# tonychang04/distributed-machine-learning-cluster

Hardware: AMD Instinct MI355X
Metric: images/sec (whole node) + p50/p95 query latency, ResNet18 ImageNet (higher is better)
Workload: dtype bf16

## Files before the change

### csrc/bindings/py_module.cpp

```cpp
#include <pybind11/numpy.h>
#include <pybind11/pybind11.h>
#include "../serve/shard.h"
#include <pybind11/stl.h>

#include <map>

#include "../kernels/kernels.h"
#include "../runtime/engine.h"
#include "../runtime/jpeg.h"
#include "../runtime/jpeg_gpu.h"
#include "../runtime/ot_io.h"

namespace py = pybind11;
using namespace dmlc;

namespace {

template <typename T>
T* P(uintptr_t v) {
  return reinterpret_cast<T*>(v);
}
hipStream_t S(uintptr_t v) { return reinterpret_cast<hipStream_t>(v); }

WeightMap to_weight_map(const py::dict& d) {
// ... 216 lines not shown
    maxpool2d(P<void>(x), P<void>(y), B, H, W, C, conv_out_dim(H, k, stride, pad),
              conv_out_dim(W, k, stride, pad), k, stride, pad, S(stream));
  });
  m.def("avgpool_global", [](uintptr_t x, uintptr_t y, int B, int HW, int C, uintptr_t stream) {
    avgpool_global(P<void>(x), P<void>(y), B, HW, C, S(stream));
  });
  m.def("avgpool_adaptive", [](uintptr_t x, uintptr_t y, int B, int H, int W, int C, int Ho, int Wo,
                               uintptr_t stream) {
    avgpool_adaptive(P<void>(x), P<void>(y), B, H, W, C, Ho, Wo, S(stream));
  });
  m.def(
      "preprocess_u8",
      [](uintptr_t x, uintptr_t y, int B, int Hin, int Win, int S_, int pad, int Wr, uintptr_t stream,
         bool paired) { preprocess_u8(P<uint8_t>(x), P<void>(y), B, Hin, Win, S_, pad, Wr, S(stream), paired); },
      py::arg("x"), py::arg("y"), py::arg("B"), py::arg("Hin"), py::arg("Win"), py::arg("S"), py::arg("pad"),
      py::arg("Wr"), py::arg("stream"), py::arg("paired") = false);
  m.attr("STEM_POOL_K") = kStemPoolK;
  m.def("stem_pool_pick_strip", &stem_pool_pick_strip);
  m.def("stem_pool_u8_pick_strip", &stem_pool_u8_pick_strip);
  m.def("conv3x3_stream_supported", &conv3x3_stream_supported, py::arg("Hin"), py::arg("Win"), py::arg("Cin"),
        py::arg("Cout"), py::arg("stride") = 1);
  m.def("conv3x3_stream", [](uintptr_t x, uintptr_t w, uintptr_t bias, uintptr_t res, uintptr_t y, uintptr_t zero,
                             int B, int H, int W, int Cin, int Cout, int stride, bool relu, uintptr_t stream,
                             uintptr_t stamps, uintptr_t wd, uintptr_t bd, uintptr_t yd, uintptr_t wfrag,
                             uintptr_t wdfrag) {
    conv3x3_stream(P<void>(x), P<void>(w), P<float>(bias), P<void>(res), P<void>(y), P<void>(zero), B, H, W, Cin, Cout,
                   stride, relu, S(stream), P<unsigned long long>(stamps), P<void>(wd), P<float>(bd), P<void>(yd),
                   P<void>(wfrag), P<void>(wdfrag));
  }, py::arg("x"), py::arg("w"), py::arg("bias"), py::arg("res"), py::arg("y"), py::arg("zero"), py::arg("B"),
        py::arg("H"), py::arg("W"), py::arg("Cin"), py::arg("Cout"), py::arg("stride"), py::arg("relu"),
        py::arg("stream"), py::arg("stamps") = 0, py::arg("wd") = 0, py::arg("bd") = 0, py::arg("yd") = 0,
        py::arg("wfrag") = 0, py::arg("wdfrag") = 0);
  m.def("conv3x3_stream_uses_frag", &conv3x3_stream_uses_frag);
  m.def("conv3x3_stream_set_variant", &conv3x3_stream_set_variant);
  m.def("conv3x3_rows_supported", &conv3x3_rows_supported);
  m.def("conv3x3_rows_pick_strip", &conv3x3_rows_pick_strip);
  m.def("conv3x3_rows", [](uintptr_t x, uintptr_t w, uintptr_t bias, uintptr_t res, uintptr_t y, uintptr_t zero,
                           int B, int H, int W, int C, bool relu, int strip, uintptr_t stream, uintptr_t wfrag) {
    conv3x3_rows(P<void>(x), P<void>(w), P<float>(bias), P<void>(res), P<void>(y), P<void>(zero), B, H, W, C, relu,
                 strip, S(stream), P<void>(wfrag));
  }, py::arg("x"), py::arg("w"), py::arg("bias"), py::arg("res"), py::arg("y"), py::arg("zero"), py::arg("B"),
        py::arg("H"), py::arg("W"), py::arg("C"), py::arg("relu"), py::arg("strip"), py::arg("stream"),
        py::arg("wfrag") = 0);
  m.def("conv3x3_block_supported", &conv3x3_block_supported);
  m.def("conv3x3_block", [](uintptr_t x, uintptr_t wf1, uintptr_t b1, uintptr_t wf2, uintptr_t b2, uintptr_t y,
                            uintptr_t zero, int B, uintptr_t stream) {
    conv3x3_block(P<void>(x), P<void>(wf1), P<float>(b1), P<void>(wf2), P<float>(b2), P<void>(y), P<void>(zero), B,
                  S(stream));
  }, py::arg("x"), py::arg("wf1"), py::arg("b1"), py::arg("wf2"), py::arg("b2"), py::arg("y"), py::arg("zero"),
        py::arg("B"), py::arg("stream"));
  m.def("bottleneck56", [](uintptr_t x, uintptr_t w1, uintptr_t a1, uintptr_t b1, uintptr_t wf2, uintptr_t b2,
                           uintptr_t wf3, uintptr_t b3, uintptr_t y, float res_scale, float out_inv_scale, int B,
                           uintptr_t stream) {
    bottleneck56(P<void>(x), P<void>(w1), P<float>(a1), P<float>(b1), P<void>(wf2), P<float>(b2), P<void>(wf3),
                 P<float>(b3), P<void>(y), res_scale, out_inv_scale, B, S(stream));
  }, py::arg("x"), py::arg("w1"), py::arg("a1"), py::arg("b1"), py::arg("wf2"), py::arg("b2"), py::arg("wf3"),
     py::arg("b3"), py::arg("y"), py::arg("res_scale"), py::arg("out_inv_scale"), py::arg("B"), py::arg("stream") = 0);
  m.def("conv3x3_stream8_supported", &conv3x3_stream8_supported);
  m.def("conv3x3_stream8_frag_offset", &conv3x3_stream8_frag_offset);
  m.def("conv3x3_stream8_set_variant", &conv3x3_stream8_set_variant);
  m.def("conv3x3_stream8", [](uintptr_t x, uintptr_t wf, uintptr_t alpha, uintptr_t bias, uintptr_t y, uintptr_t zero,
                              int B, int H, int W, int Cin, int Cout, int stride, bool relu, float out_inv_scale,
                              uintptr_t stream) {
    conv3x3_stream8(P<void>(x), P<void>(wf), P<float>(alpha), P<float>(bias), P<void>(y), P<void>(zero), B, H, W, Cin,
                    Cout, stride, relu, out_inv_scale, S(stream));
  }, py::arg("x"), py::arg("wf"), py::arg("alpha"), py::arg("bias"), py::arg("y"), py::arg("zero"), py::arg("B"),
// ... 244 lines not shown
          "from_ot",
          [](const std::string& arch, const std::string& path, int device, int num_classes, int image_size,
             const std::map<std::string, bool>& options) {
            return new Engine(arch, ot_load(path), device, num_classes, image_size, engine_options(options));
          },
          py::arg("arch"), py::arg("path"), py::arg("device") = 0, py::arg("num_classes") = 1000,
          py::arg("image_size") = 224, py::arg("options") = std::map<std::string, bool>{})
      .def("reserve", &Engine::reserve, py::call_guard<py::gil_scoped_release>())
      .def(
          "forward",
          [](Engine& e, uintptr_t images, int B, int Hin, int Win, uintptr_t idx, uintptr_t prob,
             uintptr_t logits, uintptr_t stream, bool use_graph) {
            e.forward(P<uint8_t>(images), B, Hin, Win, P<int32_t>(idx), P<float>(prob), P<float>(logits),
                      S(stream), use_graph);
          },
          py::arg("images"), py::arg("B"), py::arg("Hin"), py::arg("Win"), py::arg("idx"),
          py::arg("prob"), py::arg("logits"), py::arg("stream"), py::arg("use_graph") = true,
          py::call_guard<py::gil_scoped_release>())
      .def(
          "forward_topk",
          [](Engine& e, uintptr_t images, int B, int Hin, int Win, int k, uintptr_t idx, uintptr_t prob,
             uintptr_t logits, uintptr_t stream, bool use_graph) {
            e.forward_topk(P<uint8_t>(images), B, Hin, Win, k, P<int32_t>(idx), P<float>(prob), P<float>(logits),
                           S(stream), use_graph);
          },
          py::arg("images"), py::arg("B"), py::arg("Hin"), py::arg("Win"), py::arg("k"), py::arg("idx"),
          py::arg("prob"), py::arg("logits"), py::arg("stream"), py::arg("use_graph") = true,
          py::call_guard<py::gil_scoped_release>())
      .def("profile",
           [](Engine& e, uintptr_t images, int B, int Hin, int Win, uintptr_t stream) {
             return e.profile(P<uint8_t>(images), B, Hin, Win, S(stream));
           })
      .def("activation_ptr", [](const Engine& e, int id) { return reinterpret_cast<uintptr_t>(e.activation(id)); })
      .def("activation_shape",
           [](const Engine& e, int id) {
             auto s = e.activation_shape(id);
             return py::make_tuple(s.H, s.W, s.C, s.f32);
           })
      .def("op_list", [=](const Engine& e) { return op_list(e.ops()); })
      .def("plan", [=](const Engine& e, int B, int Hin, int Win, int topk) {
        return plan_list(e.plan_lines(e.plan(B, Hin, Win, topk)));
      }, py::arg("B"), py::arg("Hin"), py::arg("Win"), py::arg("topk") = 1)
      .def_property_readonly("num_cus", &Engine::num_cus)
      .def_property_readonly("num_activations", &Engine::num_activations)
      .def_property_readonly("arch", &Engine::arch)
      .def_property_readonly("device", &Engine::device)
      .def_property_readonly("num_classes", &Engine::num_classes)
      .def_property_readonly("image_size", &Engine::image_size)
      .def_property_readonly("max_batch", &Engine::max_batch)
      .def_property_readonly("weight_bytes", &Engine::weight_bytes)
      .def_property_readonly("activation_bytes", &Engine::activation_bytes)
      .def_property_readonly("gflop_per_image", &Engine::gflop_per_image);

  bind_dp(m);
}
```

### csrc/kernels/conv3x3_stream.hip

```cpp
#include <atomic>

#include "common.h"
#include "kernels.h"

namespace dmlc {

namespace {

template <int N>
__device__ __forceinline__ void vm_wait() {
  static_assert(N >= 0 && N < 64, "vmcnt range");
  asm volatile("s_waitcnt vmcnt(%0)" ::"i"(N) : "memory");
}

struct StreamConvArgs {
  const bf16* x;
  const bf16* w;
  const float* bias;
  const bf16* res;
  bf16* y;
  const bf16* zero;
  const bf16* wd;
  const float* bd;
  bf16* yd;
// ... 425 lines not shown
}

template <int H, int W, int CI, int CO, int HS, int IMG, int NSP, int WM, int S, bool WR = false, int PD = 4,
          int NG = 1, int PRIO = 0>
void launch_stream(const StreamConvArgs& a, hipStream_t s) {
  using G = StreamGeom<H, W, CI, HS, IMG, S, 3>;
  constexpr size_t lds = WR ? (size_t)G::XBYTES : G::LDS;
  static_assert(lds <= 160 * 1024, "LDS budget");
  const int grid = (a.B + IMG - 1) / IMG * (H / HS) * NSP;
  if constexpr (WR) {
    if constexpr (S == 2) {
      if (a.yd) {
        hipLaunchKernelGGL((conv3x3_stream_kernel<H, W, CI, CO, HS, IMG, NSP, WM, S, 3, true, true, PD, NG, PRIO>),
                           dim3(grid), dim3(512), lds, s, a);
        return;
      }
    }
      hipLaunchKernelGGL((conv3x3_stream_kernel<H, W, CI, CO, HS, IMG, NSP, WM, S, 3, false, true, PD, NG, PRIO>),
                         dim3(grid), dim3(512), lds, s, a);
    return;
  } else {
    if constexpr (S == 2) {
      if (a.yd) {
        hipLaunchKernelGGL((conv3x3_stream_kernel<H, W, CI, CO, HS, IMG, NSP, WM, S, 3, true, false>), dim3(grid),
                           dim3(512), lds, s, a);
        return;
      }
    }
    hipLaunchKernelGGL((conv3x3_stream_kernel<H, W, CI, CO, HS, IMG, NSP, WM, S, 3, false, false>), dim3(grid),
                       dim3(512), lds, s, a);
  }
}

std::atomic<int> g_stream_variant{0};

}

void conv3x3_stream_set_variant(int v) { g_stream_variant = v; }

bool conv3x3_stream_pool_supported(int Hin, int Win, int Cin, int Cout, int stride) {
  return stride == 1 && Hin == 7 && Win == 7 && Cin == 512 && Cout == 512;
}

bool conv3x3_stream_supported(int Hin, int Win, int Cin, int Cout, int stride) {
  if (stride == 1)
    return Cin == Cout && ((Hin == 28 && Win == 28 && Cin == 128) || (Hin == 14 && Win == 14 && Cin == 256) ||
                           (Hin == 7 && Win == 7 && Cin == 512) || (Hin == 56 && Win == 56 && Cin == 64));
  if (stride == 2)
    return (Cout == 2 * Cin && ((Hin == 56 && Win == 56 && Cin == 64) || (Hin == 28 && Win == 28 && Cin == 128) ||
                                (Hin == 14 && Win == 14 && Cin == 256))) ||
           (Cout == Cin && Hin == 56 && Win == 56 && Cin == 128);
  return false;
}

bool conv3x3_stream_uses_frag(int Hin, int Win, int Cin, int Cout, int stride) {
  if (stride == 2)
    return (Cout == 2 * Cin && ((Hin == 28 && Win == 28 && Cin == 128) || (Hin == 14 && Cin == 256))) ||
           (Cout == Cin && Hin == 56 && Win == 56 && Cin == 128);
  return stride == 1 && Cin == Cout && ((Hin == 7 && Win == 7 && Cin == 512) || (Hin == 14 && Win == 14 && Cin == 256));
}

void conv3x3_stream(const void* x, const void* w, const float* bias, const void* res, void* y, const void* zero,
                    int B, int Hin, int Win, int Cin, int Cout, int stride, bool relu, hipStream_t s,
                    unsigned long long* stamps, const void* wd, const float* bd, void* yd, const void* wfrag,
                    const void* wdfrag, void* pool, bool store_y, float out_inv_scale) {
  if (B <= 0) return;
  if (out_inv_scale > 0.f && (res || pool || yd || !store_y))
    throw std::invalid_argument("conv3x3_stream: e4m3 output without residual, pool or downsample only");
  if ((pool || !store_y) && !conv3x3_stream_pool_supported(Hin, Win, Cin, Cout, stride))
    throw std::invalid_argument("conv3x3_stream: fused avgpool needs whole-image workgroups");
  if (pool && ((uintptr_t)pool & 15)) throw std::invalid_argument("conv3x3_stream: misaligned pool");
  if (!conv3x3_stream_supported(Hin, Win, Cin, Cout, stride))
    throw std::invalid_argument("conv3x3_stream: unsupported shape");
  if (!x || !w || !bias || !y || !zero ||
      (((uintptr_t)x | (uintptr_t)w | (uintptr_t)y | (uintptr_t)zero | (uintptr_t)res) & 15))
    throw std::invalid_argument("conv3x3_stream: null / misaligned operand");
  StreamConvArgs a;
  a.x = (const bf16*)x;
  a.w = (const bf16*)w;
  a.bias = bias;
  a.res = (const bf16*)res;
  a.y = (bf16*)y;
  a.zero = (const bf16*)zero;
  a.B = B;
  a.relu = relu;
  a.stamps = stamps;
  a.stagger = kernel_stagger(kStagStream);
  a.wd = (const bf16*)wd;
  a.bd = bd;
  a.yd = (bf16*)yd;
  a.wf = (const bf16*)wfrag;
  a.wdf = (const bf16*)wdfrag;
// ... 52 lines not shown
```

### csrc/kernels/kernels.h

```cpp
#pragma once
#include <hip/hip_runtime.h>
#include <stdint.h>
#include <stdexcept>
#include <string>

namespace dmlc {

#define DMLC_HIP_CHECK(expr)                                                          \
  do {                                                                                \
    hipError_t _e = (expr);                                                           \
    if (_e != hipSuccess)                                                             \
      throw std::runtime_error(std::string("HIP error ") + hipGetErrorString(_e) +    \
                               " at " + __FILE__ + ":" + std::to_string(__LINE__)); \
  } while (0)

struct ConvArgs {
  const void* x = nullptr;
  const void* w = nullptr;
  const void* zero = nullptr;
  const float* bias = nullptr;
  const void* res = nullptr;
  void* y = nullptr;
  int B = 0, H = 0, W = 0, Cin = 0;
  int Ho = 0, Wo = 0, KH = 1, KW = 1, stride = 1, pad = 0;
// ... 100 lines not shown
void bottleneck56_head(const void* x, const void* w1, const float* b1, const void* wf2, const float* b2, void* y,
                       int B, hipStream_t s);
bool conv3x3_s2rows_supported(int Hin, int Win, int Cin, int Cout);
bool conv3x3_s2rows128_supported(int Hin, int Win, int Cin, int Cout);
void conv3x3_s2rows128(const void* x, const void* wf, const float* bias, void* y, int B, bool relu,
                       float out_inv_scale, hipStream_t s);
void conv3x3_s2rows(const void* x, const void* wf, const float* bias, const void* wdf, const float* bd, void* y,
                    void* yd, const void* zero, int B, bool relu, hipStream_t s);
bool conv3x3_rows28_supported(int H, int W, int Cin, int Cout);
void conv3x3_rows28(const void* x, const void* wf, const float* bias, const void* res, void* y, int B, bool relu,
                    hipStream_t s, float out_inv_scale = 0.f, const void* xds = nullptr,
                    const void* wds = nullptr, const float* bds = nullptr);
bool conv_small_supported(int H, int W, int CI, int CO, int stride);
int conv_small_pick_mf(int B, int H, int W, int CI, int CO, int stride, int num_cus);
void conv_small_set_mf(int mf);
void conv_small(const void* x, const void* wf, const float* bias, const void* res, void* y, int B, int H, int W,
                int CI, int CO, int stride, bool relu, int mf, hipStream_t s, const void* wdf = nullptr,
                const float* bd = nullptr, void* yd = nullptr);
bool conv3x3_stream_supported(int Hin, int Win, int Cin, int Cout, int stride = 1);
bool conv3x3_stream8_supported(int Hin, int Win, int Cin, int Cout, int stride = 1);
size_t conv3x3_stream8_frag_offset(int j, int t, int nf, int h, int lane, int KT);
void conv3x3_stream8(const void* x, const void* wf, const float* alpha, const float* bias, void* y, const void* zero,
                     int B, int Hin, int Win, int Cin, int Cout, int stride, bool relu, float out_inv_scale,
                     hipStream_t s);
void conv3x3_stream8_set_variant(int v);
void conv3x3_stream(const void* x, const void* w, const float* bias, const void* res, void* y, const void* zero,
                    int B, int Hin, int Win, int Cin, int Cout, int stride, bool relu, hipStream_t s,
                    unsigned long long* stamps = nullptr, const void* wd = nullptr, const float* bd = nullptr,
                    void* yd = nullptr, const void* wfrag = nullptr, const void* wdfrag = nullptr,
                    void* pool = nullptr, bool store_y = true, float out_inv_scale = 0.f);
bool conv3x3_stream_pool_supported(int Hin, int Win, int Cin, int Cout, int stride);
bool conv3x3_stream_uses_frag(int Hin, int Win, int Cin, int Cout, int stride);
void conv3x3_stream_set_variant(int v);
inline size_t stream_frag_index(int n, int k, int K) {
  const int g = n / 32, r = n % 32;
  const int nf = (r >> 2) & 1, rr = ((r >> 3) << 2) | (r & 3);
  const int t = k / 32, kk = k % 32, lane = (kk / 8) * 16 + rr, e = kk % 8;
  return ((((size_t)g * (K / 32) + t) * 2 + nf) * 64 + lane) * 8 + e;
}
int stem_pool_pick_strip(int B, int PH, int num_cus);
int stem_pool_u8_pick_strip(int B, int PH, int num_cus);
void stem_conv_pool(const void* x, const void* w, const float* bias, void* y, int B, int S, int Wq, int strip,
                    hipStream_t s);
void stem_conv_pool_set_dbg(int dbg);
void stem_conv_pool_set_stamps(void* p);
enum StaggerKernel { kStagStream = 0, kStagBlock, kStagRows28, kStagS2rows, kStagStem, kStagStream8, kStagConv1x1,
                     kStagBottleneck, kStagCount };
int kernel_stagger(int k);
void kernel_stagger_set(int k, int n);
void kernel_stagger_for_lanes(int lanes);
void stem_conv_pool_u8(const uint8_t* x, const void* w, const float* bias, void* y, int B, int S, int strip,
                       hipStream_t s, const void* w_dense = nullptr);
constexpr int kStemDenseK = 160;
struct StemDenseCell {
  int dy, u;
  bool pad;
};
constexpr StemDenseCell stem_dense_cell(int j, int fq) {
  if (j < 15) return {2 * (j / 5) + (fq & 1), 2 * (j % 5) + (fq >> 1), false};
  const int hp = 2 * (j - 15) + (fq >> 1), m = fq & 1;
  if (hp < 3) return {2 * hp + m, 10, false};
  if (hp < 6) return {m ? 5 : 6, hp - 3, m == 1};
  return {6, 3 + 2 * (hp - 6) + m, false};
}
inline int stem_dense_k_index(int dy, int dx, int c) {
  const int e = 3 * dx + c, u = e / 2, h = e % 2;
// ... 37 lines not shown
```

### csrc/runtime/engine.cpp

```cpp
#include "engine.h"

#include <algorithm>
#include <cmath>
#include <cstring>
#include <optional>
#include <stdexcept>

#include "trace.h"

namespace dmlc {

namespace {

size_t align_up(size_t v, size_t a) { return (v + a - 1) / a * a; }

const HostTensor& need(const WeightMap& w, const std::string& k) {
  auto it = w.find(k);
  if (it == w.end()) throw std::runtime_error("missing weight: " + k);
  return it->second;
}

const HostTensor* maybe(const WeightMap& w, const std::string& k) {
  auto it = w.find(k);
  return it == w.end() ? nullptr : &it->second;
// ... 18 lines not shown
  static const std::vector<float> table = [] {
    std::vector<float> t(127);
    for (int c = 0; c < 127; ++c) {
      const int e = c >> 3, m = c & 7;
      t[c] = e == 0 ? std::ldexp((float)m / 8.f, -6) : std::ldexp(1.f + (float)m / 8.f, e - 7);
    }
    return t;
  }();
  if (std::isnan(f)) return 0x7f;
  const uint8_t sign = std::signbit(f) ? 0x80 : 0;
  const float a = std::fabs(f);
  if (a >= 448.f) return sign | 0x7e;
  int c = (int)(std::upper_bound(table.begin(), table.end(), a) - table.begin()) - 1;
  if (c < 126) {
    const float lo = table[c], hi = table[c + 1];
    if (a - lo > hi - a || (a - lo == hi - a && (c & 1))) ++c;
  }
  return sign | (uint8_t)c;
}

}

bool EngineOptions::set(const std::string& name, bool v) {
  static const std::pair<const char*, bool EngineOptions::*> fields[] = {
      {"persistent", &EngineOptions::persistent},   {"fused_stem", &EngineOptions::fused_stem},
      {"fused_preprocess", &EngineOptions::fused_preprocess}, {"row_conv", &EngineOptions::row_conv},
      {"rows_wreg", &EngineOptions::rows_wreg},     {"fused_block", &EngineOptions::fused_block},
      {"fused_bottleneck", &EngineOptions::fused_bottleneck},
      {"ds_into_expand", &EngineOptions::ds_into_expand}, {"ds_into_conv2", &EngineOptions::ds_into_conv2},
      {"chain_1x1", &EngineOptions::chain_1x1},
      {"fp8_3x3_in", &EngineOptions::fp8_3x3_in},
      {"stream_conv", &EngineOptions::stream_conv}, {"stream_wreg", &EngineOptions::stream_wreg},
      {"stream_l4s2", &EngineOptions::stream_l4s2}, {"fuse_ds", &EngineOptions::fuse_ds},
      {"bigtile", &EngineOptions::bigtile},         {"fused_pool", &EngineOptions::fused_pool},
      {"fused_head", &EngineOptions::fused_head},   {"fc_small", &EngineOptions::fc_small},
      {"direct13", &EngineOptions::direct13},
      {"direct27", &EngineOptions::direct27},
      {"fork_ds", &EngineOptions::fork_ds},         {"fp8_3x3", &EngineOptions::fp8_3x3},
      {"fp8_3x3_out", &EngineOptions::fp8_3x3_out},
      {"fp8_3x3_out_s2", &EngineOptions::fp8_3x3_out_s2},
      {"conv1x1", &EngineOptions::conv1x1},         {"s2rows", &EngineOptions::s2rows},
      {"s2rows128", &EngineOptions::s2rows128},
      {"rows28", &EngineOptions::rows28},           {"stem_roles", &EngineOptions::stem_roles},
      {"stem_dense", &EngineOptions::stem_dense},
      {"fc_gemm", &EngineOptions::fc_gemm},
      {"igemm_small_m", &EngineOptions::igemm_small_m},
      {"small_conv", &EngineOptions::small_conv},
  };
  for (const auto& f : fields)
    if (name == f.first) {
      this->*(f.second) = v;
      return true;
    }
  return false;
}

Engine::Engine(const std::string& arch, const WeightMap& weights, int device, int num_classes,
               int image_size, const EngineOptions& options)
    : arch_(arch), device_(device), num_classes_(num_classes), image_size_(image_size), opt_(options) {
  if (num_classes % 4 != 0) throw std::invalid_argument("num_classes must be a multiple of 4");
  DMLC_HIP_CHECK(hipSetDevice(device_));
  hipDeviceProp_t prop;
  DMLC_HIP_CHECK(hipGetDeviceProperties(&prop, device_));
  num_cus_ = prop.multiProcessorCount;
  build_graph(weights, true);
  pack_weights(weights);
// ... 1078 lines not shown
      case Path::Rows28:
        st.kernel = Kernel::Rows28;
        if (ds_conv2 >= 0 && op.res == ops[ds_conv2].out) {
          st.ds_op = ds_conv2;
          ds_conv2 = -1;
        }
        break;
      case Path::Rows:
        st.kernel = Kernel::Rows;
        st.wreg = L.wf_off && opt.rows_wreg;
        st.count = conv3x3_rows_pick_strip(B, is.H, st.wreg ? 2 * cus : cus);
        break;
      case Path::OneByOne:
        st.kernel = Kernel::Conv1x1;
        break;
      case Path::BigTile: {
        const ConvArgs a = e.conv_geom(op, B);
        st.kernel = Kernel::BigTile;
        st.cfg = conv_bigtile_pick(a, cus);
        st.count = conv_bigtile_splits(a, st.cfg, cus);
        break;
      }
      case Path::Igemm:
        break;
      case Path::Fc: {
        if (side) break;
        const ConvArgs a = e.conv_geom(op, B);
        st.kernel = Kernel::FcGemm;
        st.count = fc_gemm_splits(a, cus);
        while (st.count > 1 && ((size_t)st.count * B * a.Npad > kSplitKWsElems || (a.Kpad / 64) % st.count))
          --st.count;
        break;
      }
    }
  }

  std::vector<Step> run(bool native, bool side, bool keep_acts, int topk) {
    const bool side_ready = side && std::find(path.begin(), path.end(), Path::BigTile) == path.end();
    for (size_t oi = 0; oi < ops.size(); oi = steps.back().first_op + steps.back().n_ops) {
      const Op& op = ops[oi];
      switch (op.type) {
        case OpType::Preprocess:
          if (native && opt.fused_preprocess && conv(oi + 1) && oi + 2 < ops.size() &&
              ops[oi + 2].type == OpType::MaxPool && convs[ops[oi + 1].conv].alex_stem)
            emit(Kernel::AlexStem, oi, 3);
          else if (native && opt.fused_preprocess && op.k == 1)
            emit(Kernel::None, oi, 1);
          else
            emit(Kernel::Preprocess, oi, 1);
          break;
        case OpType::Conv:
          plan_conv(oi, side_ready, keep_acts);
          break;
        case OpType::StemPool: {
          const ConvLayer& L = convs[op.conv];
          const int PH = shapes[op.out].H;
          if (native && opt.fused_preprocess) {
            Step& st = emit(Kernel::StemPoolU8, oi, 1);
            st.count = opt.stem_roles ? stem_pool_u8_pick_strip(B, PH, cus) : stem_pool_pick_strip(B, PH, cus);
            st.wreg = opt.stem_dense && L.wf_off;
          } else {
            emit(Kernel::StemPool, oi, 1).count = stem_pool_pick_strip(B, PH, cus);
          }
          break;
        }
        case OpType::MaxPool:
          emit(Kernel::MaxPool, oi, 1);
          break;
        case OpType::AvgPoolGlobal:
          if (pooled) {
            emit(Kernel::None, oi, 1);
            if (head_fusable(oi)) emit(Kernel::HeadPooled, oi + 1, 2);
          } else if (head_fusable(oi) && B >= kPoolThenHeadB) {
            emit(Kernel::AvgPoolGlobal, oi, 1);
            emit(Kernel::HeadPooled, oi + 1, 2);
          } else if (head_fusable(oi)) {
            emit(Kernel::HeadFused, oi, 3);
          } else {
            emit(Kernel::AvgPoolGlobal, oi, 1);
          }
          break;
        case OpType::AvgPoolAdaptive:
          emit(Kernel::AvgPoolAdaptive, oi, 1);
          break;
        case OpType::SoftmaxTop1:
          emit(Kernel::SoftmaxTop1, oi, 1);
          break;
      }
    }
    if (topk > 1) {
      Step& st = emit(Kernel::SoftmaxTopK, ops.size() - 1, 0);
      st.count = topk;
    }
    return std::move(steps);
  }
};

std::vector<Step> Engine::plan(int B, bool native, bool side, bool keep_acts, int topk) const {
  if (topk < 1 || topk > std::min(num_classes_, kMaxTopK))
    throw std::invalid_argument("top-k: k must be in 1..min(num_classes, " + std::to_string(kMaxTopK) + ")");
  return Planner(*this, B).run(native, side, keep_acts, topk);
}

std::string Engine::step_detail(const Step& st) const {
  std::string d;
  auto add = [&](const std::string& s) { d += (d.empty() ? "" : " ") + s; };
  const bool in_k = st.kernel == Kernel::Rows28 || st.kernel == Kernel::Conv1x1Cat;
  if (st.ds_op >= 0) add((in_k ? "dsk=" : "ds=") + ops_[st.ds_op].name);
  if (st.pool_op >= 0) add("pool=" + ops_[st.pool_op].name);
  if (st.wreg) add("wreg");
  if (!st.store_y) add("nostore");
  if (st.side) add("side");
  if (st.cfg >= 0) add("cfg=" + std::to_string(st.cfg));
  if (st.count > 0) {
    const char* what = st.kernel == Kernel::Small ? "mf=" : st.kernel == Kernel::SoftmaxTopK ? "k=" : (st.kernel == Kernel::BigTile || st.kernel == Kernel::FcGemm) ? "splits=" : "strip=";
    add(what + std::to_string(st.count));
  }
  return d;
}

std::vector<Engine::PlanLine> Engine::plan_lines(const std::vector<Step>& steps) const {
  std::vector<PlanLine> out;
  for (const Step& st : steps) out.push_back(PlanLine{kernel_name(st.kernel), ops_[st.first_op].name, step_detail(st), st.n_ops});
  return out;
}

void Engine::run_ops(const std::vector<Step>& steps, const uint8_t* images, int B, int Hin, int Win, int32_t* idx,
                     float* prob, float* logits, hipStream_t s, std::vector<hipEvent_t>* evs, bool trace) {
  size_t ei = 0;
  if (evs) DMLC_HIP_CHECK(hipEventRecord((*evs)[ei++], s));
  std::map<int, hipEvent_t> joined;
  const uint8_t* wa = (const uint8_t*)warena_;
  auto W = [&](size_t off) { return (const void*)(wa + off); };
  auto F = [&](size_t off) { return (const float*)(wa + off); };
  auto inv_scale = [&](int act) { return shapes_[act].fp8 ? 1.f / shapes_[act].scale : 0.f; };
  const bool topk = !steps.empty() && steps.back().kernel == Kernel::SoftmaxTopK;
  int32_t* const idx_out = (idx && !topk) ? idx : dummy_idx_;
  float* const prob_out = (prob && !topk) ? prob : (float*)(dummy_idx_ + max_batch_);
  for (const Step& st : steps) {
    const size_t oi = st.first_op;
    const Op& op = ops_[oi];
    std::optional<TraceRange> tr;
    if (trace && st.kernel != Kernel::None) tr.emplace(op.name.c_str());
    hipStream_t cs = s;
// ... 61 lines not shown
        conv1x1_chain(a, ra, num_cus_, cs);
        break;
      }
      case Kernel::Bottleneck56: {
        const ConvLayer& L = *Lp;
        const ConvLayer& L2 = convs_[ops_[oi + 1].conv];
        const ConvLayer& L3 = convs_[ops_[oi + 2].conv];
        const int y = ops_[oi + 2].out;
        bottleneck56(acts_[op.in], W(L.w_off), F(L.a_off), F(L.b_off), W(L2.wf_off), F(L2.b_off), W(L3.wf_off),
                     F(L3.b_off), acts_[y], isp->scale, 1.f / shapes_[y].scale, B, s);
        break;
      }
      case Kernel::Bottleneck56Head: {
        const ConvLayer& L2 = convs_[ops_[oi + 1].conv];
        bottleneck56_head(acts_[op.in], W(Lp->w_off), F(Lp->b_off), W(L2.wf_off), F(L2.b_off), acts_[ops_[oi + 1].out],
                          B, s);
        break;
      }
      case Kernel::Block: {
        const ConvLayer& L2 = convs_[ops_[oi + 1].conv];
        conv3x3_block(acts_[op.in], W(Lp->wf_off), F(Lp->b_off), W(L2.wf_off), F(L2.b_off), acts_[ops_[oi + 1].out],
                      zero_, B, s);
        break;
      }
      case Kernel::S2Rows:
        conv3x3_s2rows(acts_[op.in], W(Lp->wf_off), F(Lp->b_off), D ? W(D->wf_off) : nullptr,
                       D ? F(D->b_off) : nullptr, acts_[op.out], D ? acts_[d->out] : nullptr, zero_, B, Lp->relu, cs);
        break;
      case Kernel::S2Rows128:
        conv3x3_s2rows128(acts_[op.in], W(Lp->wf_off), F(Lp->b_off), acts_[op.out], B, Lp->relu, inv_scale(op.out), cs);
        break;
      case Kernel::Stream: {
        const ConvLayer& L = *Lp;
        conv3x3_stream(acts_[op.in], W(L.w_off), F(L.b_off), res, acts_[op.out], zero_, B, isp->H, isp->W, isp->C,
                       L.cout, L.stride, L.relu, cs, nullptr, D ? W(D->w_off) : nullptr, D ? F(D->b_off) : nullptr,
                       D ? acts_[d->out] : nullptr, st.wreg ? W(L.wf_off) : nullptr,
                       (st.wreg && D) ? W(D->wf_off) : nullptr, ypool, st.store_y, inv_scale(op.out));
        break;
      }
      case Kernel::Direct13:
        conv3x3_13(acts_[op.in], W(Lp->wf_off), F(Lp->b_off), acts_[op.out], zero_, B, isp->C, Lp->cout, Lp->relu, cs,
                   ypool);
        break;
      case Kernel::Direct27:
        conv5x5_27(acts_[op.in], W(Lp->wf_off), F(Lp->b_off), acts_[op.out], zero_, B, cs, ypool);
        break;
      case Kernel::Small:
        conv_small(acts_[op.in], W(Lp->wf_off), F(Lp->b_off), res, acts_[op.out], B, isp->H, isp->W, isp->C, Lp->cout,
                   Lp->stride, Lp->relu, st.count, cs, D ? W(D->wf_off) : nullptr, D ? F(D->b_off) : nullptr,
                   D ? acts_[d->out] : nullptr);
        break;
      case Kernel::Stream8:
        conv3x3_stream8(acts_[op.in], W(Lp->wf_off), F(Lp->a_off), F(Lp->b_off), acts_[op.out], zero_, B, isp->H,
                        isp->W, isp->C, Lp->cout, Lp->stride, Lp->relu, 1.f / shapes_[op.out].scale, cs);
        break;
      case Kernel::Rows28:
        if (D)
          conv3x3_rows28(acts_[op.in], W(Lp->wf_off), F(Lp->b_off), nullptr, acts_[op.out], B, Lp->relu, cs, 0.f,
                         acts_[d->in], W(D->wf_off), F(D->b_off));
        else
          conv3x3_rows28(acts_[op.in], W(Lp->wf_off), F(Lp->b_off), res, acts_[op.out], B, Lp->relu, cs,
                         inv_scale(op.out));
        break;
      case Kernel::Rows:
        conv3x3_rows(acts_[op.in], W(Lp->w_off), F(Lp->b_off), res, acts_[op.out], zero_, B, isp->H, isp->W, isp->C,
                     Lp->relu, st.count, cs, st.wreg ? W(Lp->wf_off) : nullptr);
// ... 132 lines not shown
```

### csrc/runtime/engine.h

```cpp
#pragma once
#include <hip/hip_runtime.h>

#include <map>
#include <memory>
#include <string>
#include <tuple>
#include <vector>

#include "../kernels/kernels.h"
#include "weights.h"

namespace dmlc {

enum class OpType { Preprocess, Conv, StemPool, MaxPool, AvgPoolGlobal, AvgPoolAdaptive, SoftmaxTop1 };

struct ActShape {
  int H = 0, W = 0, C = 0;
  bool f32 = false;
  bool fp8 = false;
  float scale = 1.f;
  std::vector<float> cscale;
  size_t elems_per_image() const { return (size_t)H * W * C; }
  size_t elem_bytes() const { return f32 ? 4 : fp8 ? 1 : 2; }
};
// ... 21 lines not shown

  bool plain() const { return !fp8 && !fc && !pair && !stem_pool && in_act >= 0; }
  bool plain_3x3() const { return plain() && kh == 3 && kw == 3 && pad == 1; }
  bool plain_ds2() const { return plain() && kh == 1 && kw == 1 && stride == 2 && pad == 0; }
};

struct Op {
  OpType type;
  int in = -1, out = -1, res = -1;
  int conv = -1;
  int k = 0, stride = 0, pad = 0;
  std::string name;
  bool side = false;
};

constexpr int kSmallConvMaxB = 4;
constexpr int kPoolThenHeadB = 32;

struct EngineOptions {
  bool persistent = true;
  bool igemm_small_m = true;
  bool small_conv = true;
  bool fused_stem = true;
  bool fused_preprocess = true;
  bool row_conv = true;
  bool rows_wreg = true;
  bool fused_block = true;
  bool fused_bottleneck = true;
  bool ds_into_expand = true;
  bool ds_into_conv2 = true;
  bool stream_conv = true;
  bool stream_wreg = true;
  bool stream_l4s2 = true;
  bool fuse_ds = true;
  bool s2rows128 = true;
  bool s2rows = true;
  bool rows28 = true;
  bool stem_roles = true;
  bool fc_gemm = true;
  bool stem_dense = true;
  bool bigtile = true;
  bool conv1x1 = true;
  bool chain_1x1 = true;
  bool fused_pool = true;
  bool fused_head = true;
  bool direct13 = true;
  bool direct27 = true;
  bool fc_small = true;
  bool fork_ds = false;
  bool fp8_3x3 = false;
  bool fp8_3x3_out = true;
  bool fp8_3x3_out_s2 = false;
  bool fp8_3x3_in = true;

  bool set(const std::string& name, bool value);
};

struct PackRegion {
  std::string layer, kind;
  size_t off = 0, bytes = 0;
};

constexpr size_t kSplitKWsElems = (size_t)16 << 20;

enum class Kernel {
  None,
  AlexStem, StemPoolU8, StemPool, FcSmall, Conv1x1Cat, Conv1x1Chain, Bottleneck56, Bottleneck56Head, Block,
  S2Rows, S2Rows128, Stream, Stream8, Rows28, Rows, Small, Direct13, Direct27, Conv1x1, BigTile, Igemm, FcGemm,
  HeadPooled, HeadFused, AvgPoolGlobal, AvgPoolAdaptive, MaxPool, Preprocess, SoftmaxTop1, SoftmaxTopK
};
const char* kernel_name(Kernel k);

struct Step {
  Kernel kernel = Kernel::None;
  int first_op = 0, n_ops = 1;
  int ds_op = -1;
  int pool_op = -1;
  bool wreg = false;
  bool store_y = true;
  bool side = false;
  int cfg = -1;
  int count = 0;
};

class Engine {
 public:
  Engine(const std::string& arch, const WeightMap& weights, int device, int num_classes = 1000,
         int image_size = 224, const EngineOptions& options = {});
  Engine(const Engine& src, int device);
  void copy_weights_from(const Engine& src);
  ~Engine();
  Engine& operator=(const Engine&) = delete;
  static std::vector<PackRegion> pack_audit(const std::string& arch, const WeightMap& weights,
                                            const EngineOptions& options, size_t* total,
                                            int num_classes = 1000, int image_size = 224);
  std::vector<Step> plan(int B, bool native, bool side, bool keep_acts, int topk = 1) const;
  std::vector<Step> plan(int B, int Hin, int Win, int topk = 1) const {
    return plan(B, Hin == image_size_ && Win == image_size_, opt_.fork_ds, false, topk);
  }
  std::string step_detail(const Step& st) const;
  struct PlanLine {
    std::string kernel, first_op, detail;
    int n_ops = 1;
  };
  static std::vector<PlanLine> plan_audit(const std::string& arch, const WeightMap& weights,
                                          const EngineOptions& options, int B, bool native, int num_cus,
                                          std::vector<Op>* engine_ops = nullptr, int num_classes = 1000,
                                          int image_size = 224, int topk = 1);
  std::vector<PlanLine> plan_lines(const std::vector<Step>& steps) const;
  void* weight_arena() const { return warena_; }

  const std::string& arch() const { return arch_; }
  int device() const { return device_; }
// ... 91 lines not shown
```

### distributed-machine-learning-cluster_amd/ops/__init__.py

```python
from __future__ import annotations


import torch

from .. import native


def _stream() -> int:
    return torch.cuda.current_stream().cuda_stream


def _need_cuda(*ts):
    for t in ts:
        if t is not None and not t.is_cuda:
            raise RuntimeError("dmlc.ops kernels need CUDA/HIP tensors (no CPU fallback)")


def _ptr(t):
    return 0 if t is None else t.data_ptr()


def conv_kpad(cin: int, kh: int, kw: int, stem: bool = False) -> int:
    return native().conv_kpad(cin, kh, kw, stem)

# ... 254 lines not shown
                   frag: bool | torch.Tensor = False):
    _need_cuda(x, w_packed, bias, res)
    C = native()
    B, H, W, Cin = x.shape
    Cout = w_packed.shape[0]
    if not C.conv3x3_stream_supported(H, W, Cin, Cout, stride):
        raise ValueError("conv3x3_stream: unsupported shape")
    y = torch.empty(B, H // stride, W // stride, Cout, dtype=x.dtype, device=x.device)
    stamps = 0
    if _PHASE_STAMPS:
        global BT_STAMPS
        if BT_STAMPS is None:
            BT_STAMPS = torch.zeros(1 << 16, dtype=torch.int64, device=x.device)
        stamps = _ptr(BT_STAMPS)
    yd = wd = bd = None
    if downsample is not None:
        wd, bd = downsample[0].contiguous(), downsample[1].float().contiguous()
        _need_cuda(wd, bd)
        if stride != 2 or tuple(wd.shape) != (Cout, Cin):
            raise ValueError("conv3x3_stream: downsample needs stride 2 and weights [Cout, Cin]")
        yd = torch.empty_like(y)
    wf = None
    if frag is not False and frag is not None:
        if not C.conv3x3_stream_uses_frag(H, W, Cin, Cout, stride):
            raise ValueError("conv3x3_stream: no register-weight variant for this shape")
        wf = frag if isinstance(frag, torch.Tensor) else stream_weight_frag(w_packed)
    wdf = None
    if wf is not None and wd is not None:
        wdf = downsample[2] if len(downsample) > 2 else stream_weight_frag(wd)
    C.conv3x3_stream(_ptr(x.contiguous()), _ptr(w_packed.contiguous()), _ptr(bias.float().contiguous()),
                     _ptr(None if res is None else res.contiguous()), _ptr(y), _ptr(_zero_page(x.device)), B, H, W,
                     Cin, Cout, stride, relu, _stream(), stamps, _ptr(wd), _ptr(bd), _ptr(yd), _ptr(wf), _ptr(wdf))
    return y if downsample is None else (y, yd)


FP8 = torch.float8_e4m3fn
FP8_MAX = 448.0


def quantize_fp8(t: torch.Tensor, scale: float) -> torch.Tensor:
    return (t.float() / scale).clamp(-FP8_MAX, FP8_MAX).to(FP8)


def pack_conv_weight_fp8(w: torch.Tensor, device=None) -> tuple[torch.Tensor, torch.Tensor]:
    cout, cin, kh, kw = w.shape
    kpad, npad = conv_kpad(cin, kh, kw), conv_npad(cout)
    wk = torch.zeros(npad, kpad)
    wk[:cout, : kh * kw * cin] = w.float().permute(0, 2, 3, 1).reshape(cout, -1)
    s = (wk.abs().amax(1) / FP8_MAX).clamp_min(1e-12)
    q = quantize_fp8(wk / s[:, None], 1.0)
    return (q.to(device), s.to(device)) if device is not None else (q, s)


def conv2d_fp8(x: torch.Tensor, w_q: torch.Tensor, alpha: torch.Tensor, cout: int, kh: int, kw: int,
               stride: int = 1, pad: int = 0, bias: torch.Tensor | None = None, res: torch.Tensor | None = None,
               res_scale: float = 1.0, relu: bool = False, out_scale: float | None = None,
               tile: int = -1) -> torch.Tensor:
    _need_cuda(x, w_q, alpha, bias, res)
    C = native()
    B, H, W, Cin = x.shape
    in8 = x.dtype == FP8
    Ho, Wo = C.conv_out_dim(H, kh, stride, pad), C.conv_out_dim(W, kw, stride, pad)
    out8 = out_scale is not None
    y = torch.empty(B, Ho, Wo, cout, device=x.device, dtype=FP8 if out8 else torch.bfloat16)
    if bias is not None:
        bias = bias.float().contiguous()
# ... 332 lines not shown
```

Measured before the change: 297,400.

## Chain consecutive 14x14 stream 3x3 convs in one persistent kernel via LDS

```diff
diff --git a/csrc/bindings/py_module.cpp b/csrc/bindings/py_module.cpp
--- a/csrc/bindings/py_module.cpp
+++ b/csrc/bindings/py_module.cpp
@@ -272,6 +272,24 @@
         py::arg("stream"), py::arg("stamps") = 0, py::arg("wd") = 0, py::arg("bd") = 0, py::arg("yd") = 0,
         py::arg("wfrag") = 0, py::arg("wdfrag") = 0);
   m.def("conv3x3_stream_uses_frag", &conv3x3_stream_uses_frag);
+  m.attr("STREAM_CHAIN_MAX") = kStreamChainMax;
+  m.def("conv3x3_stream_chain_supported", &conv3x3_stream_chain_supported);
+  m.def("conv3x3_stream_chain", [](uintptr_t x, uintptr_t zero, int B,
+                                   const std::vector<std::tuple<uintptr_t, uintptr_t, uintptr_t, uintptr_t, bool>>& phases,
+                                   uintptr_t stream, uintptr_t stamps) {
+    std::vector<StreamChainPhase> ph;
+    for (const auto& [wf, bias, res, y, relu] : phases) {
+      StreamChainPhase q;
+      q.wf = P<void>(wf);
+      q.bias = P<float>(bias);
+      q.res = P<void>(res);
+      q.y = P<void>(y);
+      q.relu = relu;
+      ph.push_back(q);
+    }
+    conv3x3_stream_chain(P<void>(x), P<void>(zero), B, ph.data(), (int)ph.size(), S(stream),
+                         P<unsigned long long>(stamps));
+  }, py::arg("x"), py::arg("zero"), py::arg("B"), py::arg("phases"), py::arg("stream"), py::arg("stamps") = 0);
   m.def("conv3x3_stream_set_variant", &conv3x3_stream_set_variant);
   m.def("conv3x3_rows_supported", &conv3x3_rows_supported);
   m.def("conv3x3_rows_pick_strip", &conv3x3_rows_pick_strip);
@@ -582,6 +600,9 @@
              return e.profile(P<uint8_t>(images), B, Hin, Win, S(stream));
            })
       .def("activation_ptr", [](const Engine& e, int id) { return reinterpret_cast<uintptr_t>(e.activation(id)); })
+      .def("copy_activation", [](const Engine& e, int id, uintptr_t dst, size_t bytes, uintptr_t stream) {
+        DMLC_HIP_CHECK(hipMemcpyAsync(P<void>(dst), e.activation(id), bytes, hipMemcpyDeviceToDevice, S(stream)));
+      })
       .def("activation_shape",
            [](const Engine& e, int id) {
              auto s = e.activation_shape(id);
diff --git a/csrc/kernels/conv3x3_stream.hip b/csrc/kernels/conv3x3_stream.hip
--- a/csrc/kernels/conv3x3_stream.hip
+++ b/csrc/kernels/conv3x3_stream.hip
@@ -481,6 +481,216 @@
   }
 }
 
+struct ChainPhase {
+  const bf16* wf;
+  const float* bias;
+  const bf16* res;
+  bf16* y;
+  int relu;
+  int pad_;
+};
+struct StreamChainArgs {
+  const bf16* x;
+  const bf16* zero;
+  unsigned long long* stamps;
+  int B, P, stagger;
+  ChainPhase ph[kStreamChainMax];
+};
+
+template <int PD>
+__global__ __launch_bounds__(512, 1) void conv3x3_stream_chain_kernel(StreamChainArgs a) {
+  constexpr int H = 14, W = 14, CI = 256, CO = 256, WM = 2, NG = 2;
+  using G = StreamGeom<H, W, CI, H, 1, 1, 3>;
+  constexpr int BK = 32, NPIX = H * W, MFT = (NPIX + 15) / 16, MF = (MFT + WM - 1) / WM, WN = 32 * NG, NF = 2 * NG;
+  constexpr int PXB = G::PXB, ROWB = G::ROWB, ZB = G::ZB;
+  constexpr int CPX = CI / 8, XI = W * CPX / 64, KT = 9 * CI / BK, CT = CI / BK;
+  static_assert(CT % PD == 0 && MF + NF <= 15 && PXB == CO * 2, "geometry");
+
+  extern __shared__ __attribute__((aligned(16))) uint4 smem[];
+  char* xs = (char*)smem;
+
+  const int tid = threadIdx.x, lane = tid & 63;
+  const int wave = __builtin_amdgcn_readfirstlane(tid >> 6);
+  const int wm = wave % WM, wc = wave / WM;
+  const int b = blockIdx.x;
+  const int ch0 = wc * WN;
+  const bf16* img = a.x + (long)b * NPIX * CI;
+  const int P = a.P;
+  unsigned long long* const stamps = a.stamps;
+  asm volatile("" ::"s"(P), "s"(stamps));
+  start_stagger(a.stagger);
+
+  for (int k = wave; k < H * XI; k += 8) {
+    const int i = k / XI, j = k - i * XI;
+    const int ci = j * 64 + lane;
+    const int x = ci / CPX, pp = ci - x * CPX;
+    const int pc = pp ^ xswz<CPX>(i * W + x);
+    dma16(img + ((long)i * W + x) * CI + 8 * pc, xs + i * ROWB + j * 1024);
+  }
+  if (wave == 0 && lane < CPX) dma16(a.zero, xs + ZB);
+
+  int xoff[MF], ln = lane;
+#pragma unroll
+  for (int f = 0; f < MF; ++f) {
+    const int p = min(16 * (wm * MF + f) + (lane & 15), NPIX - 1);
+    const int prow = p / W, pcol = p - prow * W;
+    xoff[f] = p * PXB | (prow == 0 ? 1 : 0) | (prow == H - 1 ? 2 : 0) | (pcol == 0 ? 4 : 0) | (pcol == W - 1 ? 8 : 0);
+    asm volatile("" : "+v"(xoff[f]));
+  }
+#pragma nounroll
+  for (int q = 0; q < P; ++q) {
+    const bf16* const wfp = a.ph[q].wf;
+    const float* const bias = a.ph[q].bias;
+    const bf16* const res = a.ph[q].res;
+    bf16* const y = a.ph[q].y;
+    const int relu = a.ph[q].relu;
+    asm volatile("" ::"s"(wfp), "s"(bias), "s"(res), "s"(y), "s"(relu));
+    const bool last = q + 1 == P;
+    asm volatile("" : "+v"(ln));
+#pragma unroll
+    for (int f = 0; f < MF; ++f) asm volatile("" : "+v"(xoff[f]));
+    const int fr = ln & 15, fq = ln >> 4;
+    int xa[MF], tsw = 0;
+    auto set_tap = [&](int tap) __attribute__((always_inline)) {
+      const int kh = tap / 3, kw = tap - kh * 3;
+      const int tm = (kh == 0 ? 1 : 0) | (kh == 2 ? 2 : 0) | (kw == 0 ? 4 : 0) | (kw == 2 ? 8 : 0);
+      const int toff = ((kh - 1) * W + kw - 1) * PXB;
+#pragma unroll
+      for (int f = 0; f < MF; ++f) xa[f] = (xoff[f] & tm) ? ZB : (xoff[f] & ~15) + toff;
+      tsw = (fq << 4) ^ (xswz<CPX>(fr + (kh - 1) * W + kw - 1) << 4);
+    };
+    auto xread = [&](int f, int cc) __attribute__((always_inline)) {
+      return *(const bf16x8*)(xs + xa[f] + (tsw ^ (cc * BK * 2)));
+    };
+    unsigned long long t_start = 0, t_first = 0, t_loop = 0;
+    if (stamps) {
+      t_start = __builtin_amdgcn_s_memrealtime();
+      asm volatile("" ::"s"(t_start));
+    }
+    const __amdgpu_buffer_rsrc_t wrs = wave_rsrc(wfp + (long)(ch0 / 32) * KT * 2 * 512, NG * KT * 2 * 1024);
+    auto wfrag = [&](int t, int nf) __attribute__((always_inline)) {
+      return __builtin_bit_cast(bf16x8, __builtin_amdgcn_raw_buffer_load_b128(
+                                            wrs, ln * 16, ((nf >> 1) * KT * 2 + t * 2 + (nf & 1)) * 1024, 0));
+    };
+    bf16x8 wq[PD][NF];
+#pragma unroll
+    for (int t = 0; t < PD - 1; ++t)
+#pragma unroll
+      for (int nf = 0; nf < NF; ++nf) wq[t][nf] = wfrag(t, nf);
+    floatx4 acc[MF][NF];
+#pragma unroll
+    for (int f = 0; f < MF; ++f)
+#pragma unroll
+      for (int nf = 0; nf < NF; ++nf) acc[f][nf] = floatx4{0.f, 0.f, 0.f, 0.f};
+    set_tap(0);
+    if (q == 0)
+      vm_wait<(PD - 1) * NF>();
+    else
+      asm volatile("s_waitcnt lgkmcnt(0)" ::: "memory");
+    __builtin_amdgcn_s_barrier();
+    asm volatile("" ::: "memory");
+    if (stamps) {
+      t_first = __builtin_amdgcn_s_memrealtime();
+      asm volatile("" ::"s"(t_first));
+    }
+    bf16x8 xf[MF];
+#pragma unroll
+    for (int f = 0; f < MF; ++f) xf[f] = xread(f, 0);
+    for (int tap = 0; tap < 9; ++tap) {
+#pragma unroll
+      for (int cc = 0; cc < CT; ++cc) {
+        const int t = tap * CT + cc;
+        if (t + PD - 1 < KT)
+#pragma unroll
+          for (int nf = 0; nf < NF; ++nf) wq[(cc + PD - 1) % PD][nf] = wfrag(t + PD - 1, nf);
+        if (cc + 1 == CT && tap + 1 < 9) set_tap(tap + 1);
+        const int cn = cc + 1 == CT ? 0 : cc + 1;
+        __builtin_amdgcn_s_waitcnt(0xC07F);
+#pragma unroll
+        for (int f = 0; f < MF; ++f) {
+#pragma unroll
+          for (int nf = 0; nf < NF; ++nf)
+            acc[f][nf] = __builtin_amdgcn_mfma_f32_16x16x32_bf16(wq[cc % PD][nf], xf[f], acc[f][nf], 0, 0, 0);
+          xf[f] = xread(f, cn);
+        }
+#pragma unroll
+        for (int f = 0; f < MF; ++f) {
+          __builtin_amdgcn_sched_group_barrier(0x008, NF, 0);
+          __builtin_amdgcn_sched_group_barrier(0x100, 1, 0);
+        }
+      }
+    }
+    if (stamps) {
+      t_loop = __builtin_amdgcn_s_memrealtime();
+      asm volatile("" ::"s"(t_loop));
+    }
+
+    __builtin_amdgcn_fence(__ATOMIC_ACQ_REL, "workgroup");
+    int xo[MF];
+#pragma unroll
+    for (int f = 0; f < MF; ++f) xo[f] = xoff[f] & ~15;
+    const int er = fr, eq = fq;
+    const long ib = (long)b * NPIX * CO * 2;
+    const uint32_t cb = (uint32_t)(ch0 + 8 * eq) * 2;
+    float bs[NG][8];
+#pragma unroll
+    for (int j = 0; j < NG; ++j)
+#pragma unroll
+      for (int e = 0; e < 8; ++e) bs[j][e] = bias[ch0 + 32 * j + 8 * eq + e];
+    uint4 rv[MF][NG];
+    if (res) {
+      const char* rb = (const char*)res + ib;
+#pragma unroll
+      for (int f = 0; f < MF; ++f)
+#pragma unroll
+        for (int j = 0; j < NG; ++j) rv[f][j] = *(const uint4*)(rb + (uint32_t)(xo[f] + cb + 64 * j));
+    } else {
+#pragma unroll
+      for (int f = 0; f < MF; ++f)
+#pragma unroll
+        for (int j = 0; j < NG; ++j) rv[f][j] = make_uint4(0, 0, 0, 0);
+    }
+    if (!last) {
+      asm volatile("s_waitcnt lgkmcnt(0)" ::: "memory");
+      __builtin_amdgcn_s_barrier();
+      asm volatile("" ::: "memory");
+    }
+    const int lsw = xswz<CPX>(er);
+    char* const yb = (char*)y + ib;
+#pragma unroll
+    for (int f = 0; f < MF; ++f) {
+      const int p = 16 * (wm * MF + f) + er;
+      if (p >= NPIX) continue;
+#pragma unroll
+      for (int j = 0; j < NG; ++j) {
+        float v[8];
+#pragma unroll
+        for (int e = 0; e < 4; ++e) {
+          v[e] = acc[f][2 * j][e] + bs[j][e];
+          v[4 + e] = acc[f][2 * j + 1][e] + bs[j][4 + e];
+        }
+        if (res) {
+          float r[8];
+          unpack8(rv[f][j], r);
+#pragma unroll
+          for (int e = 0; e < 8; ++e) v[e] += r[e];
+        }
+        const uint4 packed = pack8_relu(v, relu);
+        if (y) *(uint4*)(yb + (uint32_t)(xo[f] + cb + 64 * j)) = packed;
+        if (!last) *(uint4*)(xs + xo[f] + ((((ch0 + 32 * j) / 8 + eq) ^ lsw) << 4)) = packed;
+      }
+    }
+    if (stamps && tid == 0) {
+      asm volatile("s_waitcnt vmcnt(0)" ::: "memory");
+      unsigned long long* sp = stamps + ((long)blockIdx.x * P + q) * 4;
+      sp[0] = t_start;
+      sp[1] = t_first;
+      sp[2] = t_loop;
+      sp[3] = __builtin_amdgcn_s_memrealtime();
+    }
+  }
+}
+
 std::atomic<int> g_stream_variant{0};
 
 }
@@ -507,6 +717,36 @@
     return (Cout == 2 * Cin && ((Hin == 28 && Win == 28 && Cin == 128) || (Hin == 14 && Cin == 256))) ||
            (Cout == Cin && Hin == 56 && Win == 56 && Cin == 128);
   return stride == 1 && Cin == Cout && ((Hin == 7 && Win == 7 && Cin == 512) || (Hin == 14 && Win == 14 && Cin == 256));
+}
+
+bool conv3x3_stream_chain_supported(int Hin, int Win, int Cin, int Cout, int stride) {
+  return stride == 1 && Hin == 14 && Win == 14 && Cin == 256 && Cout == 256;
+}
+
+void conv3x3_stream_chain(const void* x, const void* zero, int B, const StreamChainPhase* phases, int P,
+                          hipStream_t s, unsigned long long* stamps) {
+  if (B <= 0) return;
+  if (P < 2 || P > kStreamChainMax || !phases) throw std::invalid_argument("conv3x3_stream_chain: 2..12 phases");
+  if (!x || !zero || (((uintptr_t)x | (uintptr_t)zero) & 15))
+    throw std::invalid_argument("conv3x3_stream_chain: null / misaligned operand");
+  StreamChainArgs a{};
+  a.x = (const bf16*)x;
+  a.zero = (const bf16*)zero;
+  a.stamps = stamps;
+  a.B = B;
+  a.P = P;
+  a.stagger = kernel_stagger(kStagStream);
+  for (int q = 0; q < P; ++q) {
+    const StreamChainPhase& p = phases[q];
+    if (!p.wf || !p.bias || (q + 1 == P && !p.y) ||
+        (((uintptr_t)p.wf | (uintptr_t)p.res | (uintptr_t)p.y) & 15) || ((uintptr_t)p.bias & 3))
+      throw std::invalid_argument("conv3x3_stream_chain: null / misaligned phase operand");
+    a.ph[q] = ChainPhase{(const bf16*)p.wf, p.bias, (const bf16*)p.res, (bf16*)p.y, p.relu ? 1 : 0, 0};
+  }
+  using G = StreamGeom<14, 14, 256, 14, 1, 1, 3>;
+  static_assert(G::XBYTES <= 160 * 1024, "LDS budget");
+  hipLaunchKernelGGL((conv3x3_stream_chain_kernel<4>), dim3(B), dim3(512), (size_t)G::XBYTES, s, a);
+  DMLC_HIP_CHECK(hipGetLastError());
 }
 
 void conv3x3_stream(const void* x, const void* w, const float* bias, const void* res, void* y, const void* zero,
diff --git a/csrc/kernels/kernels.h b/csrc/kernels/kernels.h
--- a/csrc/kernels/kernels.h
+++ b/csrc/kernels/kernels.h
@@ -156,6 +156,17 @@
 bool conv3x3_stream_pool_supported(int Hin, int Win, int Cin, int Cout, int stride);
 bool conv3x3_stream_uses_frag(int Hin, int Win, int Cin, int Cout, int stride);
 void conv3x3_stream_set_variant(int v);
+constexpr int kStreamChainMax = 12;
+struct StreamChainPhase {
+  const void* wf = nullptr;
+  const float* bias = nullptr;
+  const void* res = nullptr;
+  void* y = nullptr;
+  bool relu = true;
+};
+bool conv3x3_stream_chain_supported(int Hin, int Win, int Cin, int Cout, int stride);
+void conv3x3_stream_chain(const void* x, const void* zero, int B, const StreamChainPhase* phases, int P,
+                          hipStream_t s, unsigned long long* stamps = nullptr);
 inline size_t stream_frag_index(int n, int k, int K) {
   const int g = n / 32, r = n % 32;
   const int nf = (r >> 2) & 1, rr = ((r >> 3) << 2) | (r & 3);
diff --git a/csrc/runtime/engine.cpp b/csrc/runtime/engine.cpp
--- a/csrc/runtime/engine.cpp
+++ b/csrc/runtime/engine.cpp
@@ -74,6 +74,7 @@
       {"fp8_3x3_in", &EngineOptions::fp8_3x3_in},
       {"stream_conv", &EngineOptions::stream_conv}, {"stream_wreg", &EngineOptions::stream_wreg},
       {"stream_l4s2", &EngineOptions::stream_l4s2}, {"fuse_ds", &EngineOptions::fuse_ds},
+      {"stream_chain", &EngineOptions::stream_chain},
       {"bigtile", &EngineOptions::bigtile},         {"fused_pool", &EngineOptions::fused_pool},
       {"fused_head", &EngineOptions::fused_head},   {"fc_small", &EngineOptions::fc_small},
       {"direct13", &EngineOptions::direct13},
@@ -1218,6 +1219,40 @@
           --st.count;
         break;
       }
+    }
+  }
+
+  bool chain_step(size_t si) const {
+    const Step& st = steps[si];
+    if (st.kernel != Kernel::Stream || !st.wreg || st.n_ops != 1 || st.ds_op >= 0 || st.pool_op >= 0 || st.side ||
+        !st.store_y)
+      return false;
+    const Op& op = ops[st.first_op];
+    const ConvLayer& L = convs[op.conv];
+    const ActShape& is = shapes[op.in];
+    return !shapes[op.out].fp8 && conv3x3_stream_chain_supported(is.H, is.W, is.C, L.cout, L.stride);
+  }
+
+  void mark_chains(bool keep_acts) {
+    for (size_t i = 0; i < steps.size();) {
+      size_t n = 0;
+      while (i + n < steps.size() && n < (size_t)kStreamChainMax && chain_step(i + n) &&
+             (n == 0 || ops[steps[i + n].first_op].in == ops[steps[i + n - 1].first_op].out))
+        ++n;
+      if (n < 2) {
+        ++i;
+        continue;
+      }
+      for (size_t j = 0; j < n; ++j) {
+        Step& st = steps[i + j];
+        st.chain = steps[i].first_op;
+        if (j + 1 < n && !keep_acts) {
+          const int out = ops[st.first_op].out;
+          const size_t next = steps[i + j + 1].first_op;
+          st.lds = only_reader(out, next) && ops[next].res != out;
+        }
+      }
+      i += n;
     }
   }
 
@@ -1274,6 +1309,7 @@
           break;
       }
     }
+    if (opt.stream_chain) mark_chains(keep_acts);
     if (topk > 1) {
       Step& st = emit(Kernel::SoftmaxTopK, ops.size() - 1, 0);
       st.count = topk;
@@ -1296,6 +1332,8 @@
   if (st.pool_op >= 0) add("pool=" + ops_[st.pool_op].name);
   if (st.wreg) add("wreg");
   if (!st.store_y) add("nostore");
+  if (st.chain >= 0) add("chain=" + ops_[st.chain].name);
+  if (st.lds) add("lds");
   if (st.side) add("side");
   if (st.cfg >= 0) add("cfg=" + std::to_string(st.cfg));
   if (st.count > 0) {
@@ -1423,6 +1461,22 @@
         break;
       case Kernel::Stream: {
         const ConvLayer& L = *Lp;
+        if (st.chain >= 0 && !evs) {
+          if (st.chain != (int)oi) break;
+          StreamChainPhase ph[kStreamChainMax];
+          int P = 0;
+          for (const Step* sp = &st; sp != steps.data() + steps.size() && sp->chain == st.chain; ++sp, ++P) {
+            const Op& o = ops_[sp->first_op];
+            const ConvLayer& Lq = convs_[o.conv];
+            ph[P].wf = W(Lq.wf_off);
+            ph[P].bias = F(Lq.b_off);
+            ph[P].res = o.res >= 0 ? acts_[o.res] : nullptr;
+            ph[P].y = sp->lds ? nullptr : acts_[o.out];
+            ph[P].relu = Lq.relu;
+          }
+          conv3x3_stream_chain(acts_[op.in], zero_, B, ph, P, cs);
+          break;
+        }
         conv3x3_stream(acts_[op.in], W(L.w_off), F(L.b_off), res, acts_[op.out], zero_, B, isp->H, isp->W, isp->C,
                        L.cout, L.stride, L.relu, cs, nullptr, D ? W(D->w_off) : nullptr, D ? F(D->b_off) : nullptr,
                        D ? acts_[d->out] : nullptr, st.wreg ? W(L.wf_off) : nullptr,
diff --git a/csrc/runtime/engine.h b/csrc/runtime/engine.h
--- a/csrc/runtime/engine.h
+++ b/csrc/runtime/engine.h
@@ -77,6 +77,7 @@
   bool stream_conv = true;
   bool stream_wreg = true;
   bool stream_l4s2 = true;
+  bool stream_chain = true;
   bool fuse_ds = true;
   bool s2rows128 = true;
   bool s2rows = true;
@@ -124,6 +125,8 @@
   bool wreg = false;
   bool store_y = true;
   bool side = false;
+  int chain = -1;
+  bool lds = false;
   int cfg = -1;
   int count = 0;
 };
diff --git a/distributed-machine-learning-cluster_amd/ops/__init__.py b/distributed-machine-learning-cluster_amd/ops/__init__.py
--- a/distributed-machine-learning-cluster_amd/ops/__init__.py
+++ b/distributed-machine-learning-cluster_amd/ops/__init__.py
@@ -310,6 +310,39 @@
                      _ptr(None if res is None else res.contiguous()), _ptr(y), _ptr(_zero_page(x.device)), B, H, W,
                      Cin, Cout, stride, relu, _stream(), stamps, _ptr(wd), _ptr(bd), _ptr(yd), _ptr(wf), _ptr(wdf))
     return y if downsample is None else (y, yd)
+
+
+def conv3x3_stream_chain(x: torch.Tensor, phases: list, stamps: bool = False) -> list:
+    C = native()
+    B, H, W, Cin = x.shape
+    if not C.conv3x3_stream_chain_supported(H, W, Cin, 256, 1) or not 2 <= len(phases) <= C.STREAM_CHAIN_MAX:
+        raise ValueError("conv3x3_stream_chain: [B,14,14,256] and 2..12 convs")
+    x = x.contiguous()
+    keep, outs, table = [], [], []
+    for q, (w, bias, res, relu, store) in enumerate(phases):
+        wf = (w if w.dim() == 5 else stream_weight_frag(w)).contiguous()
+        bias = bias.float().contiguous()
+        if isinstance(res, int):
+            if not 0 <= res < q or outs[res] is None:
+                raise ValueError("conv3x3_stream_chain: a residual index names an earlier, stored conv")
+            res = outs[res]
+        elif res is not None:
+            res = res.contiguous()
+            if tuple(res.shape) != tuple(x.shape):
+                raise ValueError("conv3x3_stream_chain: residual shape")
+        _need_cuda(x, wf, bias, res)
+        y = torch.empty_like(x) if store or q + 1 == len(phases) else None
+        keep += [wf, bias, res]
+        outs.append(y)
+        table.append((_ptr(wf), _ptr(bias), _ptr(res), _ptr(y), bool(relu)))
+    sp = 0
+    if stamps:
+        global BT_STAMPS
+        if BT_STAMPS is None or BT_STAMPS.numel() < 4 * B * len(phases):
+            BT_STAMPS = torch.zeros(max(1 << 16, 4 * B * len(phases)), dtype=torch.int64, device=x.device)
+        sp = _ptr(BT_STAMPS)
+    C.conv3x3_stream_chain(_ptr(x), _ptr(_zero_page(x.device)), B, table, _stream(), sp)
+    return outs
 
 
 FP8 = torch.float8_e4m3fn
```

Measured after the change: 301,800, median of 6. +1.5%, better.
